# wuyakuma/HIPRT-Path-Tracer

Hardware: AMD Instinct MI355X
Metric: Mray/s + Msample/s, Bistro 1920×1080, 1/2/4/8 MI355X; RMSE vs ref @256spp (higher is better)
Workload: dtype f32

## Files before the change

### hiprt-path-tracer_amd/csrc/mpt_kernels.hip

```cpp
#include <hip/hip_runtime.h>

#include <cfloat>
#include <cstring>
#include <initializer_list>
#include <type_traits>
#include <utility>

#include "dev_bsdf.h"
#include "mpt_internal.h"

namespace mpt {

constexpr int TB = TRAV_BLOCK;
constexpr int MAX_BOUNDARY_SKIPS = 16;
#ifndef MPT_TRACE_REFILL
#define MPT_TRACE_REFILL 32
#endif
#ifndef MPT_TRACE_BUDGET
#define MPT_TRACE_BUDGET 16
#endif
constexpr int TRACE_REFILL = MPT_TRACE_REFILL;
constexpr int TRACE_BUDGET = MPT_TRACE_BUDGET;
#ifndef MPT_TRACE_CHUNK
#define MPT_TRACE_CHUNK 256
#endif
constexpr int TRACE_CHUNK = MPT_TRACE_CHUNK;
static_assert(TRACE_CHUNK >= 64, "a refill of up to 64 lanes must fit in one new chunk");
#ifndef MPT_TRI_POSTPONE
#define MPT_TRI_POSTPONE 3
#endif
constexpr int TRI_POSTPONE = MPT_TRI_POSTPONE;
constexpr uint32_t TRI_GROUP = 0x80000000u;
constexpr int LDS_STACK = TRAV_LDS_STACK;
constexpr int SPILL_DEPTH = TRAV_SPILL_DEPTH;

DEV int lane_id() { return __lane_id(); }
DEV size_t nq_index(const DevPaths& P, int id) { return (size_t)(id & 3) * (size_t)P.nq_stride + (size_t)(id >> 2); }
DEV size_t rq_phys(const DevPaths& P, int id) {
    const int s = id / RS_RPP_HOST;
    return (size_t)(id - s * RS_RPP_HOST) * (size_t)P.n + (size_t)s;
}
DEV size_t rq_rec_at(const DevPaths& P, int s, int k) { return (size_t)k * (size_t)P.n + (size_t)s; }
DEV int wave_append(int32_t* counter, bool pred) {
    unsigned long long m = __ballot(pred);
    unsigned long long act = __ballot(1);
    int leader = __ffsll((long long)act) - 1;
    int cnt = __popcll(m);
    int base = 0;
    if (lane_id() == leader && cnt) base = atomicAdd(counter, cnt);
    base = __shfl(base, leader);
    unsigned long long lower = m & ((1ull << lane_id()) - 1ull);
    return base + __popcll(lower);
}

struct THit { int prim; float t, u, v; };

DEV uint32_t alpha_key(uint32_t pixel_seed, int bounce, int kind, int iter) {
    return wang_hash(pixel_seed ^ wang_hash((uint32_t)(bounce * 8 + kind) * 0x85EBCA77u + (uint32_t)iter * 0xC2B2AE3Du + 1u));
}
DEV float alpha_uniform(uint32_t key, int prim) {
    uint32_t h = wang_hash(key ^ ((uint32_t)prim * 0x9E3779B1u));
    h = wang_hash(h + 0x7F4A7C15u);
    return (float)(h >> 8) * (1.0f / 16777216.0f);
}
DEV bool alpha_rejects(const DevScene& S, int prim, float u, float v, uint32_t key);

#ifndef MPT_TRAV_PK
#define MPT_TRAV_PK 1
#endif
DEV uint32_t qbyte(uint32_t w0, uint32_t w1, int s) { return ((s < 4 ? w0 : w1) >> ((s & 3) * 8)) & 0xffu; }

template <bool ANY, bool STATS, bool TIE = false>
struct Trav {
    v3 o, d;
    float ix, iy, iz;
    int xr;
    float best;
    int bprim;
    float bu, bv;
    uint32_t bcls;
    uint32_t gbase, gimask, gk;
    int sp;
    int last_hit;
    uint32_t akey;
    bool alpha_on;
    int tie;

    DEV void init(v3 o_, v3 d_, int lh, float tmax, bool al, uint32_t key) {
        o = o_;
        d = d_;
        ix = 1.0f / (fabsf(d.x) > 1e-30f ? d.x : copysignf(1e-30f, d.x));
        iy = 1.0f / (fabsf(d.y) > 1e-30f ? d.y : copysignf(1e-30f, d.y));
        iz = 1.0f / (fabsf(d.z) > 1e-30f ? d.z : copysignf(1e-30f, d.z));
        int oct = (d.x > 0.0f ? 1 : 0) | (d.y > 0.0f ? 2 : 0) | (d.z > 0.0f ? 4 : 0);
        xr = oct ^ 7;
        best = ANY ? tmax : INFINITY;
        bprim = -1;
        bu = 0.0f;
        bv = 0.0f;
        bcls = 0u;
        gbase = 0;
        gimask = 1u;
        gk = 1u << (0 ^ xr);
        sp = 0;
        last_hit = lh;
        akey = key;
        alpha_on = al;
    }

    DEV void push(uint2* lds, uint32_t* spill, uint2 e) {
        if (sp < LDS_STACK) lds[sp * TB + threadIdx.x] = e;
        else { spill[2 * (sp - LDS_STACK)] = e.x; spill[2 * (sp - LDS_STACK) + 1] = e.y; }
        ++sp;
    }

    DEV bool run(const DevScene& S, const Node8* bvh_nodes, const TriRec* bvh_tris, uint2* lds, uint32_t* spill, int budget,
                 uint32_t& n_nodes, uint32_t& n_tris, uint32_t* n_slots = nullptr) {
        const float4* nodes = reinterpret_cast<const float4*>(bvh_nodes);
        const float4* tris = reinterpret_cast<const float4*>(bvh_tris);
        const int tid = threadIdx.x;
        uint32_t tbase = 0u, tmask = 0u;
        while (true) {
            if (gk == 0) {
                if (sp == 0) return true;
                if (budget <= 0) return false;
                --sp;
                uint2 e;
                if (sp < LDS_STACK) e = lds[sp * TB + tid];
                else { e.x = spill[2 * (sp - LDS_STACK)]; e.y = spill[2 * (sp - LDS_STACK) + 1]; }
                if (e.y & TRI_GROUP) { tbase = e.x; tmask = e.y & ~TRI_GROUP; }
                else { gbase = e.x; gimask = e.y & 0xffu; gk = e.y >> 8; }
            } else if (budget <= 0) {
                return false;
            }
            if (gk != 0) {
                --budget;
                int k = __builtin_ctz(gk);
                gk &= gk - 1u;
                int s = k ^ xr;
                uint32_t ni = gbase + (uint32_t)__builtin_popcount(gimask & ((1u << s) - 1u));
                if (gk) push(lds, spill, make_uint2(gbase, gimask | (gk << 8)));
                if (STATS) {
                    n_nodes++;
                    if (n_slots && lane_id() == __ffsll((long long)__ballot(1)) - 1) n_slots[0] += 64;
                }
                const float4 n0 = nodes[5 * (size_t)ni + 0];
                const float4 n1 = nodes[5 * (size_t)ni + 1];
                const float4 n2 = nodes[5 * (size_t)ni + 2];
                const float4 n3 = nodes[5 * (size_t)ni + 3];
                const float4 n4 = nodes[5 * (size_t)ni + 4];
                uint32_t eb = __float_as_uint(n0.w);
                float sx = __uint_as_float((eb & 0xffu) << 23), sy = __uint_as_float(((eb >> 8) & 0xffu) << 23),
                      sz = __uint_as_float(((eb >> 16) & 0xffu) << 23);
                uint32_t imask = eb >> 24;
                float ax = (n0.x - o.x) * ix, ay = (n0.y - o.y) * iy, az = (n0.z - o.z) * iz;
                float cx = sx * ix, cy = sy * iy, cz = sz * iz;
                uint32_t lox0 = __float_as_uint(n2.x), lox1 = __float_as_uint(n2.y);
                uint32_t loy0 = __float_as_uint(n2.z), loy1 = __float_as_uint(n2.w);
                uint32_t loz0 = __float_as_uint(n3.x), loz1 = __float_as_uint(n3.y);
                uint32_t hix0 = __float_as_uint(n3.z), hix1 = __float_as_uint(n3.w);
                uint32_t hiy0 = __float_as_uint(n4.x), hiy1 = __float_as_uint(n4.y);
                uint32_t hiz0 = __float_as_uint(n4.z), hiz1 = __float_as_uint(n4.w);
                uint32_t nx0 = ix >= 0.0f ? lox0 : hix0, nx1 = ix >= 0.0f ? lox1 : hix1;
                uint32_t fx0 = ix >= 0.0f ? hix0 : lox0, fx1 = ix >= 0.0f ? hix1 : lox1;
                uint32_t ny0 = iy >= 0.0f ? loy0 : hiy0, ny1 = iy >= 0.0f ? loy1 : hiy1;
                uint32_t fy0 = iy >= 0.0f ? hiy0 : loy0, fy1 = iy >= 0.0f ? hiy1 : loy1;
                uint32_t nz0 = iz >= 0.0f ? loz0 : hiz0, nz1 = iz >= 0.0f ? loz1 : hiz1;
                uint32_t fz0 = iz >= 0.0f ? hiz0 : loz0, fz1 = iz >= 0.0f ? hiz1 : loz1;
                uint32_t meta0 = __float_as_uint(n1.z), meta1 = __float_as_uint(n1.w);
                uint32_t hit_internal = 0u;
                uint32_t hit_tris = 0u;
#if MPT_TRAV_PK
                typedef float pf2 __attribute__((ext_vector_type(2)));
#pragma unroll
                for (int c2 = 0; c2 < 8; c2 += 2) {
                    float tn2[2], tf2[2];
#pragma unroll
                    for (int j = 0; j < 2; j++) {
                        const int c = c2 + j;
                        const pf2 qx = {(float)qbyte(nx0, nx1, c), (float)qbyte(fx0, fx1, c)};
                        const pf2 qy = {(float)qbyte(ny0, ny1, c), (float)qbyte(fy0, fy1, c)};
                        const pf2 qz = {(float)qbyte(nz0, nz1, c), (float)qbyte(fz0, fz1, c)};
                        const pf2 px = __builtin_elementwise_fma(qx, (pf2){cx, cx}, (pf2){ax, ax});
                        const pf2 py = __builtin_elementwise_fma(qy, (pf2){cy, cy}, (pf2){ay, ay});
                        const pf2 pz = __builtin_elementwise_fma(qz, (pf2){cz, cz}, (pf2){az, az});
                        tn2[j] = fmaxf(fmaxf(px.x, py.x), fmaxf(pz.x, 0.0f));
                        tf2[j] = fminf(fminf(px.y, py.y), fminf(pz.y, best));
                    }
                    const pf2 tfw = (pf2){tf2[0], tf2[1]} * (pf2){1.0000009f, 1.0000009f};
#pragma unroll
                    for (int j = 0; j < 2; j++) {
                        const int c = c2 + j;
                        bool h = tn2[j] <= tfw[j];
                        bool internal = (imask >> c) & 1u;
                        if (h && internal) hit_internal |= 1u << (c ^ xr);
                        const uint32_t mw = c < 4 ? meta0 : meta1, msh = 8u * (c & 3);
                        uint32_t lm;
                        asm("v_bfm_b32 %0, %1, %2" : "=v"(lm) : "v"((mw >> (msh + 5u)) & 7u), "v"(mw >> msh));
                        if (h) hit_tris |= lm;
                    }
                }
#else
#pragma unroll
                for (int c = 0; c < 8; c++) {
                    float tnx = fmaf((float)qbyte(nx0, nx1, c), cx, ax), tfx = fmaf((float)qbyte(fx0, fx1, c), cx, ax);
                    float tny = fmaf((float)qbyte(ny0, ny1, c), cy, ay), tfy = fmaf((float)qbyte(fy0, fy1, c), cy, ay);
                    float tnz = fmaf((float)qbyte(nz0, nz1, c), cz, az), tfz = fmaf((float)qbyte(fz0, fz1, c), cz, az);
                    float tn = fmaxf(fmaxf(tnx, tny), fmaxf(tnz, 0.0f));
                    float tf = fminf(fminf(tfx, tfy), fminf(tfz, best)) * 1.0000009f;
                    bool h = tn <= tf;
                    uint32_t meta = qbyte(meta0, meta1, c);
                    bool internal = (imask >> c) & 1u;
                    if (h && internal) hit_internal |= 1u << (c ^ xr);
                    if (h && !internal) hit_tris |= ((1u << (meta >> 5)) - 1u) << (meta & 31u);
                }
#endif
                if (hit_tris) {
                    tbase = __float_as_uint(n1.y);
                    tmask = hit_tris;
                }
                gbase = __float_as_uint(n1.x);
                gimask = imask;
                gk = hit_internal;
            }
            const int n_act = __popcll(__ballot(1));
            while (tmask) {
                if (__popcll(__ballot(1)) * TRI_POSTPONE < n_act) {
                    push(lds, spill, make_uint2(tbase, tmask | TRI_GROUP));
                    tmask = 0u;
                    break;
                }
                const uint32_t ti = tbase + (uint32_t)__builtin_ctz(tmask);
                tmask &= tmask - 1u;
                if (STATS) {
                    n_tris++;
                    if (n_slots && lane_id() == __ffsll((long long)__ballot(1)) - 1) n_slots[1] += 64;
                }
                const float4 t0 = tris[3 * (size_t)ti + 0];
                const float4 t1 = tris[3 * (size_t)ti + 1];
                const float4 t2 = tris[3 * (size_t)ti + 2];
                int prim = (int)__float_as_uint(t0.w);
                v3 e1 = mk3(t1.x, t1.y, t1.z), e2 = mk3(t2.x, t2.y, t2.z);
                v3 h = cross(d, e2);
                float a = dot(e1, h);
                if (a > -0.0000001f && a < 0.0000001f) continue;
                float f = 1.0f / a;
                v3 sv = o - mk3(t0.x, t0.y, t0.z);
                float u = f * dot(sv, h);
                if (u < 0.0f || u > 1.0f) continue;
                v3 q = cross(sv, e1);
                float v = f * dot(d, q);
                if (v < 0.0f || u + v > 1.0f) continue;
                float t = f * dot(e2, q);
                if (!(t > 0.0000001f)) continue;
                if (prim == last_hit) continue;
                const bool nearer = ANY ? (t < best || (TIE && t == best && prim < tie))
                                        : (t < best || (t == best && prim < bprim));
                if (alpha_on && __float_as_uint(t1.w) != 0u && nearer && alpha_rejects(S, prim, u, v, akey))
                    continue;
                if (ANY) {
                    if (nearer) {
                        bprim = prim; best = t; bu = u; bv = v;
                        gk = 0u; sp = 0;
                        return true;
                    }
                } else if (t < best || (t == best && prim < bprim)) {
                    best = t; bprim = prim; bu = u; bv = v; bcls = __float_as_uint(t2.w);
                }
            }
        }
    }
};

template <bool ANY, bool STATS>
DEV bool traverse(const DevScene& S, v3 o, v3 d, int last_hit, float tmax, THit& out, uint2* lds, uint32_t* spill,
                  uint32_t& n_nodes, uint32_t& n_tris, bool alpha_on = false, uint32_t akey = 0u) {
    Trav<ANY, STATS> tr;
    tr.init(o, d, last_hit, tmax, alpha_on, akey);
    tr.run(S, S.nodes, S.tris, lds, spill, 0x7fffffff, n_nodes, n_tris);
    out.prim = tr.bprim;
    out.t = tr.best;
    out.u = tr.bu;
    out.v = tr.bv;
    return tr.bprim >= 0;
}

enum TraceMode { TM_PATH = 0, TM_NEE_ANY = 1, TM_NEE_CLOSEST = 2, TM_RAW_CLOSEST = 3, TM_RAW_ANY = 4, TM_NEE_LIGHT = 5,
                 TM_NEE_LIGHT_OCC = 6, TM_LIST_ANY = 7, TM_LIST_CLOSEST = 8 };
constexpr int trace_stage(int mode) {
    return mode == TM_LIST_ANY ? TM_RAW_ANY : mode == TM_LIST_CLOSEST ? TM_RAW_CLOSEST : mode >= TM_NEE_LIGHT ? TM_NEE_CLOSEST : mode;
}

struct TraceArgs {
    DevScene S;
    DevPaths P;
    const int32_t* queue;
    const int32_t* count_ptr;
    int count_const;
    int32_t* fetch;
    const float4* raw_o;
    const float4* raw_d;
    float4* raw_hit;
    uint8_t* raw_occ;
    const uint32_t* raw_key;
    const MptFrame* F;
    int bounce;
    int alpha;
    int static_grid;
    int ext;
};
DEV uint32_t slot_pixel(const MptFrame& F, int slot, int& x, int& y);
DEV uint32_t pixel_seed(const MptFrame& F, uint32_t pix);
DEV uint32_t camera_seed(const MptFrame& F, uint32_t pix);
DEV uint32_t path_seed(const MptFrame* Fp, const DevPaths& P, int slot, bool camera);

template <int MODE, bool STATS>
__global__ __launch_bounds__(TB) __attribute__((amdgpu_waves_per_eu(
    MODE == TM_PATH ? MPT_TRACE_WAVES_PATH : (MODE == TM_LIST_ANY || MODE == TM_LIST_CLOSEST) ? MPT_TRACE_WAVES_LIST : MPT_TRACE_WAVES)))
    void k_trace(TraceArgs A) {
    __shared__ uint2 lds[LDS_STACK * TB];
    const DevScene& S = A.S;
    const DevPaths& P = A.P;
    const int count = (MODE == TM_RAW_CLOSEST || MODE == TM_RAW_ANY) ? A.count_const : *A.count_ptr;
    if (MODE == TM_NEE_LIGHT && A.static_grid && (int)(blockIdx.x * TB) >= count) return;
    uint32_t* spill = P.stack_spill + (MODE == TM_NEE_LIGHT && A.static_grid ? 0 : ((size_t)blockIdx.x * TB + threadIdx.x) * (2 * SPILL_DEPTH));
    uint32_t n_nodes = 0, n_tris = 0, n_rays = 0;
    uint32_t n_slots[2] = {0u, 0u};
    constexpr bool ANY = (MODE == TM_NEE_ANY || MODE == TM_RAW_ANY || MODE == TM_NEE_LIGHT_OCC || MODE == TM_LIST_ANY);
    constexpr bool TIE = MODE == TM_NEE_LIGHT_OCC;
    const Node8* bvh_nodes = MODE == TM_NEE_LIGHT ? S.nodes_light : S.nodes;
    const TriRec* bvh_tris = MODE == TM_NEE_LIGHT ? S.tris_light : S.tris;
    Trav<ANY, STATS, TIE> tr;
    const int n_waves = (int)gridDim.x * (TB / 64);
    const int wave_id = (int)blockIdx.x * (TB / 64) + (int)(threadIdx.x >> 6);
    int sc = (count + n_waves - 1) / max(1, n_waves);
    sc = min(TRACE_CHUNK, max(64, (sc + 63) & ~63));
    const int n_static = (int)min((long long)count, (long long)sc * n_waves);
    bool alive = false;
    bool exhausted = false;
    int ray = 0;
    int skips = 0;
    uint32_t pseed = 0u;
    bool was_inside = false;
    float qmax = 0.0f;
    int chunk_next = min(wave_id * sc, n_static);
    int chunk_end = min(chunk_next + sc, n_static);
    bool counter_done = n_static >= count;
    while (true) {
        const unsigned long long idle = __ballot(!alive);
        if (!exhausted && __popcll(idle) >= (unsigned)TRACE_REFILL) {
            const int need = __popcll(idle);
            int base = 0;
            if (MODE == TM_NEE_LIGHT && A.static_grid) {
                base = (int)(blockIdx.x * TB + (threadIdx.x & ~63u));
                exhausted = true;
            }
            int take0 = need, base1 = 0;
            if (!(MODE == TM_NEE_LIGHT && A.static_grid)) {
                base = chunk_next;
                take0 = min(need, chunk_end - chunk_next);
                chunk_next += take0;
                if (take0 < need && !counter_done) {
                    int b = 0;
                    if (lane_id() == 0) b = n_static + atomicAdd(A.fetch, TRACE_CHUNK);
                    b = __shfl(b, 0);
                    counter_done = b + TRACE_CHUNK >= count;
                    chunk_end = min(b + TRACE_CHUNK, count);
                    base1 = b;
                    chunk_next = min(b + (need - take0), chunk_end);
                } else {
                    base1 = count;
                }
                exhausted = counter_done && chunk_next >= chunk_end;
            }
            if (!alive) {
                const int r = __popcll(idle & ((1ull << lane_id()) - 1ull));
                const int i = r < take0 ? base + r : base1 + (r - take0);
                if (i < count) {
                    alive = true;
                    n_rays++;
                    float4 ro, rd;
                    if (MODE == TM_PATH) {
                        ray = A.queue ? A.queue[i] : i;
                        ro = ld_s(&P.ray_o[ray]);
                        rd = ld_s(&P.ray_d[ray]);
                        skips = 0;
                        was_inside = false;
                        if (A.alpha)
                            pseed = A.bounce == 0 ? P.seeds[ray].x : P.seeds[ray].y;
                        tr.init(mk3(ro.x, ro.y, ro.z), mk3(rd.x, rd.y, rd.z), (int)__float_as_uint(ro.w), INFINITY,
                                A.alpha != 0, A.alpha ? alpha_key(pseed, A.bounce, 0, 0) : 0u);
                    } else if (MODE == TM_NEE_ANY || MODE == TM_NEE_CLOSEST || MODE == TM_NEE_LIGHT || MODE == TM_NEE_LIGHT_OCC) {
                        if (A.ext) ray = MODE == TM_NEE_LIGHT_OCC ? P.xl_light[i] : MODE == TM_NEE_ANY ? P.xl_any[i] : P.xl_cl[i];
                        else ray = MODE == TM_NEE_LIGHT_OCC ? P.nq_light[i]
                                                            : P.nq_tgt[MODE == TM_NEE_ANY ? (size_t)i : (size_t)P.n * 3 + i];
                        ro = A.ext ? P.xq_o[ray] : ld_s(&P.nq_o[nq_index(P, ray)]);
                        rd = A.ext ? P.xq_d[ray] : ld_s(&P.nq_d[nq_index(P, ray)]);
                        qmax = rd.w;
                        const bool al = A.alpha != 0;
                        uint32_t akey = 0u;
                        if (al) akey = A.ext ? alpha_key(P.seeds[ray / P.x_per].y, A.bounce, MODE == TM_NEE_ANY ? 1 : 4, 0)
                                             : alpha_key(P.seeds[ray >> 2].y, A.bounce, (ray & 3) + 1, 0);
                        float tmax = ANY ? rd.w : INFINITY;
                        if (TIE) {
                            const float4 h = A.ext ? P.xq_hit[ray] : P.nhit[ray >> 2];
                            tmax = h.x;
                            tr.tie = (int)__float_as_uint(h.w);
                        }
                        tr.init(mk3(ro.x, ro.y, ro.z), mk3(rd.x, rd.y, rd.z), (int)__float_as_uint(ro.w), tmax, al, akey);
                        if (MODE == TM_NEE_LIGHT && S.n_light_tris == 0) tr.gk = 0u;
                    } else if (MODE == TM_LIST_ANY || MODE == TM_LIST_CLOSEST) {
                        ray = (int)rq_phys(P, A.queue[i]);
                        ro = A.raw_o[ray];
                        rd = A.raw_d[ray];
                        tr.init(mk3(ro.x, ro.y, ro.z), mk3(rd.x, rd.y, rd.z), (int)__float_as_uint(ro.w), ANY ? rd.w : INFINITY,
                                A.alpha != 0, A.alpha ? A.raw_key[ray] : 0u);
                    } else {
                        ray = i;
                        ro = A.raw_o[i];
                        rd = A.raw_d[i];
                        tr.init(mk3(ro.x, ro.y, ro.z), mk3(rd.x, rd.y, rd.z), (int)__float_as_uint(ro.w), ANY ? rd.w : INFINITY, false, 0u);
                    }
                }
            }
        }
        if (__ballot(alive) == 0) {
            if (exhausted) break;
            continue;
        }
        if (!alive) continue;
        if (!tr.run(S, bvh_nodes, bvh_tris, lds, spill, TRACE_BUDGET, n_nodes, n_tris, STATS ? n_slots : nullptr)) continue;
        const bool found = tr.bprim >= 0;
        if (MODE == TM_PATH) {
            VState vs = vs_load_s(P.vsA, P.vsB, ray);
            bool again = false;
            if (found) {
                was_inside = vs.pos > 0;
                if (was_inside) vs.dist += tr.best;
                int mi = S.mat_idx[tr.bprim];
                bool skip = vs_push(vs, mi, S.mat_prio[mi]);
                if (skip && ++skips < MAX_BOUNDARY_SKIPS) {
                    vs.dist += tr.best;
                    again = true;
                }
            }
            vs_store_s(P.vsA, P.vsB, ray, vs);
            if (again) {
                n_rays++;
                tr.init(tr.o + tr.best * tr.d, tr.d, tr.last_hit, INFINITY, A.alpha != 0,
                        A.alpha ? alpha_key(pseed, A.bounce, 0, skips) : 0u);
                continue;
            }
            st_s(&P.ray_o[ray], make_float4(tr.o.x, tr.o.y, tr.o.z, __uint_as_float((uint32_t)tr.last_hit)));
            st_s(&P.hit[ray], make_float4(tr.best, tr.bu, tr.bv, __uint_as_float((uint32_t)(found ? tr.bprim : -1))));
            st_s(&P.hit_inside[ray], (uint8_t)(was_inside ? 1 : 0));
            st_s(&P.hit_cls[ray], found ? (uint8_t)tr.bcls : (uint8_t)0xffu);
        } else if (MODE == TM_NEE_ANY) {
            if (A.ext) P.xq_occ[ray] = found ? 1 : 0;
            else st_s(&P.occ[nq_index(P, ray)], (uint8_t)(found ? 1 : 0));
        } else if (MODE == TM_NEE_CLOSEST || MODE == TM_NEE_LIGHT) {
            bool ok = found && tr.best < qmax;
            (A.ext ? P.xq_hit[ray] : P.nhit[ray >> 2]) =
                make_float4(tr.best, tr.bu, tr.bv, __uint_as_float((uint32_t)(ok ? tr.bprim : -1)));
            if (MODE == TM_NEE_LIGHT && ok) {
                if (A.ext) P.xl_light[atomicAdd(&P.counters[CTR_XLIGHT], 1)] = ray;
                else P.nq_light[atomicAdd(&P.counters[CTR_LIGHT], 1)] = ray;
            }
        } else if (MODE == TM_NEE_LIGHT_OCC) {
            if (found) (A.ext ? P.xq_hit[ray] : P.nhit[ray >> 2]).w = __uint_as_float(0xffffffffu);
        } else if (MODE == TM_RAW_ANY || MODE == TM_LIST_ANY) {
            A.raw_occ[ray] = found ? 1 : 0;
        } else {
            A.raw_hit[ray] = make_float4(tr.best, tr.bu, tr.bv, __uint_as_float((uint32_t)(found ? tr.bprim : -1)));
        }
        alive = false;
    }
    if (STATS) {
        for (int off = 32; off > 0; off >>= 1) {
            n_nodes += __shfl_xor(n_nodes, off);
            n_tris += __shfl_xor(n_tris, off);
            n_rays += __shfl_xor(n_rays, off);
            n_slots[0] += __shfl_xor(n_slots[0], off);
            n_slots[1] += __shfl_xor(n_slots[1], off);
        }
        if (lane_id() == 0) {
            unsigned long long* st = (unsigned long long*)&P.stats[trace_stage(MODE) * STATS_STRIDE];
            atomicAdd(st + 0, (unsigned long long)n_rays);
            atomicAdd(st + 1, (unsigned long long)n_nodes);
            atomicAdd(st + 2, (unsigned long long)n_tris);
            atomicAdd(st + 4, (unsigned long long)n_slots[0]);
            atomicAdd(st + 5, (unsigned long long)n_slots[1]);
        }
    }
}

DEV v3 ld3(const float* p, int i) { return mk3(p[3 * (size_t)i], p[3 * (size_t)i + 1], p[3 * (size_t)i + 2]); }
DEV v2 ld2(const float* p, int i) { return mk2(p[2 * (size_t)i], p[2 * (size_t)i + 1]); }
DEV int3 tri_idx(const DevScene& S, int p) { return make_int3(S.idx[3 * (size_t)p], S.idx[3 * (size_t)p + 1], S.idx[3 * (size_t)p + 2]); }
DEV v3 uv_interp3(const float* data, int3 t, v2 uv) { return ld3(data, t.y) * uv.x + ld3(data, t.z) * uv.y + ld3(data, t.x) * (1.0f - uv.x - uv.y); }
DEV v2 uv_interp2(const float* data, int3 t, v2 uv) { return ld2(data, t.y) * uv.x + ld2(data, t.z) * uv.y + ld2(data, t.x) * (1.0f - uv.x - uv.y); }
DEV v3 tri_normal(const DevScene& S, int p) {
    const float4* tr = reinterpret_cast<const float4*>(S.tris);
    (void)tr;
    int3 t = tri_idx(S, p);
    v3 A = ld3(S.pos, t.x), B = ld3(S.pos, t.y), C = ld3(S.pos, t.z);
    return normalize(cross(B - A, C - A));
}
DEV void tex_rgba(const DevScene& S, int ti, bool srgb, v2 uv, float out[4]) {
    int w = S.tex_dims[2 * ti], h = S.tex_dims[2 * ti + 1];
    float u = wrap01(uv.x), v = 1.0f - wrap01(uv.y);
    int x = (int)(u * (float)(w - 1)), y = (int)(v * (float)(h - 1));
    const uint8_t* p = S.tex + S.tex_off[ti] + (size_t)(x + y * w) * 4;
    uchar4 c = *reinterpret_cast<const uchar4*>(p);
    if (srgb) {
        out[0] = S.srgb[c.x]; out[1] = S.srgb[c.y]; out[2] = S.srgb[c.z]; out[3] = S.srgb[c.w];
        return;
    }
    out[0] = (float)c.x / 255.0f; out[1] = (float)c.y / 255.0f; out[2] = (float)c.z / 255.0f; out[3] = (float)c.w / 255.0f;
}
DEV bool has_tex(int ti) { return ti != MPT_NO_TEXTURE && ti != MPT_CONSTANT_EMISSIVE_TEXTURE; }
DEV v2 attr_tc(const DevScene& S, int prim, v2 uv) {
    const float4* r = S.tri_attr + 5 * (size_t)prim;
    const float4 c = r[2], d = r[3];
    return mk2(c.w, d.x) * uv.x + mk2(d.y, d.z) * uv.y + mk2(c.y, c.z) * (1.0f - uv.x - uv.y);
}
DEV bool alpha_rejects(const DevScene& S, int prim, float u, float v, uint32_t key) {
    const Mat& m = S.mats[S.mat_idx[prim]];
    float a = 1.0f;
    if (S.n_tex > 0 && has_tex(m.base_color_texture_index)) {
        v2 tc = attr_tc(S, prim, mk2(u, v));
        float r[4];
        tex_rgba(S, m.base_color_texture_index, true, tc, r);
        a = r[3];
    }
    float comp = m.alpha_opacity * a;
    return !(alpha_uniform(key, prim) < comp);
}
DEV void prop_f(const DevScene& S, float& v, v2 uv, int ti) { if (has_tex(ti)) { float r[4]; tex_rgba(S, ti, false, uv, r); v = r[0]; } }
DEV void prop_c(const DevScene& S, MptColor& v, v2 uv, int ti) { if (has_tex(ti)) { float r[4]; tex_rgba(S, ti, false, uv, r); v.r = r[0]; v.g = r[1]; v.b = r[2]; } }

DEV Col emission_of(const Mat& m) { return C3(m.emission) * m.emission_strength; }
DEV bool is_emissive(const Mat& m) {
    float k = m.emission_strength;
    return !is_zero(m.emission.r * k) || !is_zero(m.emission.g * k) || !is_zero(m.emission.b * k) || m.emissive_texture_used;
}

DEV Mat intersection_material(const DevScene& S, int mi, v2 uv, bool white_furnace) {
    Mat m = S.mats[mi];
    MptColor e;
    e.r = m.emission.r * m.emission_strength / m.emission_strength;
    e.g = m.emission.g * m.emission_strength / m.emission_strength;
    e.b = m.emission.b * m.emission_strength / m.emission_strength;
    if (S.n_tex > 0) prop_c(S, e, uv, m.emission_texture_index);
    m.emission = e;
    if (white_furnace) { m.base_color.r = 1.0f; m.base_color.g = 1.0f; m.base_color.b = 1.0f; }
    else if (S.n_tex > 0 && has_tex(m.base_color_texture_index)) {
        float r[4];
        tex_rgba(S, m.base_color_texture_index, true, uv, r);
        m.base_color.r = r[0]; m.base_color.g = r[1]; m.base_color.b = r[2];
    }
    if (S.n_tex > 0) {
        if (m.roughness_metallic_texture_index != MPT_NO_TEXTURE) {
            float r[4];
            tex_rgba(S, m.roughness_metallic_texture_index, false, uv, r);
            m.roughness = r[1];
            m.metallic = r[2];
        } else {
            prop_f(S, m.metallic, uv, m.metallic_texture_index);
            prop_f(S, m.roughness, uv, m.roughness_texture_index);
        }
        prop_f(S, m.oren_nayar_sigma, uv, m.oren_sigma_texture_index);
        prop_f(S, m.specular, uv, m.specular_texture_index);
        prop_f(S, m.specular_tint, uv, m.specular_tint_texture_index);
        prop_c(S, m.specular_color, uv, m.specular_color_texture_index);
        prop_f(S, m.anisotropy, uv, m.anisotropic_texture_index);
        prop_f(S, m.anisotropy_rotation, uv, m.anisotropic_rotation_texture_index);
        prop_f(S, m.coat, uv, m.coat_texture_index);
        prop_f(S, m.coat_roughness, uv, m.coat_roughness_texture_index);
        prop_f(S, m.coat_ior, uv, m.coat_ior_texture_index);
        prop_f(S, m.sheen, uv, m.sheen_texture_index);
        prop_f(S, m.sheen_roughness, uv, m.sheen_roughness_texture_index);
        prop_c(S, m.sheen_color, uv, m.sheen_color_texture_index);
        prop_f(S, m.specular_transmission, uv, m.specular_transmission_texture_index);
    }
    float coat = m.coat;
    m.emissive_texture_used = m.emission_texture_index > 0;
    float tbr = sqrtf(sqrtf(minr(1.0f, pow4(m.roughness) + 2.0f * pow4(m.coat_roughness))));
    m.roughness = lerpr(m.roughness, lerpr(m.roughness, tbr, coat), m.coat_roughening);
    float tsr = sqrtf(sqrtf(minr(1.0f, pow4(m.second_roughness) + 2.0f * pow4(m.coat_roughness))));
    m.second_roughness = lerpr(m.second_roughness, lerpr(m.second_roughness, tsr, coat), m.coat_roughening);
    return m;
}

DEV v3 normal_mapped(const DevScene& S, const Mat& m, v3 n, int p, v2 tc) {
    int3 t = tri_idx(S, p);
    v2 d1 = ld2(S.uv, t.y) - ld2(S.uv, t.x), d2 = ld2(S.uv, t.z) - ld2(S.uv, t.x);
    v3 e1 = ld3(S.pos, t.y) - ld3(S.pos, t.x), e2 = ld3(S.pos, t.z) - ld3(S.pos, t.x);
    float di = 1.0f / (d1.x * d2.y - d1.y * d2.x);
    v3 T = (e1 * d2.y - e2 * d1.y) * di;
    v3 B = (e2 * d1.x - e1 * d2.x) * di;
    float r[4];
    tex_rgba(S, m.normal_map_texture_index, false, tc, r);
    v3 ts = normalize(mk3(r[0] - 0.5f, r[1] - 0.5f, r[2] - 0.5f));
    return to_world(normalize(T), normalize(B), n, ts);
}
DEV v3 shading_normal_of(const DevScene& S, v3 gn, int p, v2 uv, v2 tc) {
    int3 t = tri_idx(S, p);
    const Mat& m = S.mats[S.mat_idx[p]];
    v3 n = S.has_n[t.x] ? normalize(uv_interp3(S.nrm, t, uv)) : gn;
    if (S.n_tex > 0 && m.normal_map_texture_index != MPT_NO_TEXTURE) n = normal_mapped(S, m, n, p, tc);
    return n;
}

struct HitAttr { v2 tc; v3 gn, sn; int mi; };
DEV HitAttr hit_attributes(const DevScene& S, int prim, v2 uv) {
    const float4* r = S.tri_attr + 5 * (size_t)prim;
    const float4 a = r[0], b = r[1], c = r[2], d = r[3], e = r[4];
    const v3 n0 = mk3(a.x, a.y, a.z), n1 = mk3(a.w, b.x, b.y), n2 = mk3(b.z, b.w, c.x);
    const v2 t0 = mk2(c.y, c.z), t1 = mk2(c.w, d.x), t2 = mk2(d.y, d.z);
    HitAttr h;
    h.tc = t1 * uv.x + t2 * uv.y + t0 * (1.0f - uv.x - uv.y);
    h.gn = normalize(mk3(e.x, e.y, e.z));
    h.mi = __float_as_int(e.w);
    v3 n = __float_as_uint(d.w) ? normalize(n1 * uv.x + n2 * uv.y + n0 * (1.0f - uv.x - uv.y)) : h.gn;
    if (S.n_tex > 0) {
        const Mat& m = S.mats[h.mi];
        if (m.normal_map_texture_index != MPT_NO_TEXTURE) n = normal_mapped(S, m, n, prim, h.tc);
    }
    h.sn = n;
    return h;
}
#ifndef MPT_TU_PART
__global__ void k_tri_attr(DevScene S, float4* out) {
    const int p = blockIdx.x * blockDim.x + threadIdx.x;
    if (p >= S.n_tris) return;
    const int3 t = tri_idx(S, p);
    const v3 n0 = ld3(S.nrm, t.x), n1 = ld3(S.nrm, t.y), n2 = ld3(S.nrm, t.z);
    const v2 t0 = ld2(S.uv, t.x), t1 = ld2(S.uv, t.y), t2 = ld2(S.uv, t.z);
    const v3 g = tri_normal(S, p);
    float4* r = out + 5 * (size_t)p;
    r[0] = make_float4(n0.x, n0.y, n0.z, n1.x);
    r[1] = make_float4(n1.y, n1.z, n2.x, n2.y);
    r[2] = make_float4(n2.z, t0.x, t0.y, t1.x);
    r[3] = make_float4(t1.y, t2.x, t2.y, __uint_as_float(S.has_n[t.x] ? 1u : 0u));
    r[4] = make_float4(g.x, g.y, g.z, __int_as_float(S.mat_idx[p]));
}

#endif
DEV uint32_t slot_pixel(const MptFrame& F, int slot, int& x, int& y) {
    int r = slot / F.res_x;
    x = slot - r * F.res_x;
    int bh = F.band_height;
    y = ((r / bh) * F.band_count + F.band_index) * bh + (r % bh);
    return (uint32_t)x + (uint32_t)y * (uint32_t)F.res_x;
}
DEV uint32_t pixel_seed(const MptFrame& F, uint32_t pix, uint32_t random_seed) {
    const MptRenderSettings& rs = F.render_settings;
    return rs.freeze_random ? wang_hash(pix + 1u) : wang_hash((pix + 1u) * (uint32_t)(rs.sample_number + 1) * random_seed);
}
DEV uint32_t pixel_seed(const MptFrame& F, uint32_t pix) { return pixel_seed(F, pix, F.random_seed); }
DEV uint32_t camera_seed(const MptFrame& F, uint32_t pix) {
    return pixel_seed(F, pix, F.camera_random_seed ? F.camera_random_seed : F.random_seed);
}
DEV int bounce_lss(const MptFrame& F, int bounce) {
    const int lss = F.options.direct_light_sampling;
    if (lss != MPT_LSS_RESTIR_DI || bounce == 0) return lss;
    switch (F.options.restir_di_later_bounces_sampling_strategy) {
    case MPT_RESTIR_DI_LATER_BOUNCES_UNIFORM_ONE_LIGHT: return MPT_LSS_UNIFORM_ONE_LIGHT;
    case MPT_RESTIR_DI_LATER_BOUNCES_BSDF: return MPT_LSS_BSDF;
    case MPT_RESTIR_DI_LATER_BOUNCES_MIS_LIGHT_BSDF: return MPT_LSS_MIS_LIGHT_BSDF;
    default: return MPT_LSS_RIS_BSDF_AND_LIGHT;
    }
}
DEV void batch_split(const DevPaths& P, int slot, int& pix, int& sub) {
    if (P.batch == 1) { pix = slot; sub = 0; return; }
    const int g = P.group;
    const int q = slot / g;
    const int grp = q / P.batch;
    sub = q - grp * P.batch;
    pix = grp * g + (slot - q * g);
}
DEV int batch_slot(const DevPaths& P, int pix, int sub) {
    const int g = P.group;
    const int grp = pix / g;
    return (grp * P.batch + sub) * g + (pix - grp * g);
}
DEV uint32_t path_seed(const MptFrame* Fp, const DevPaths& P, int slot, bool camera) {
    int pix, sub;
    batch_split(P, slot, pix, sub);
    const MptFrame& F = Fp[sub];
    int x, y;
    const uint32_t gpix = slot_pixel(F, pix, x, y);
    return camera ? camera_seed(F, gpix) : pixel_seed(F, gpix);
}

DEV bool has_adaptive_buffers(const MptRenderSettings& rs) {
    return (rs.stop_pixel_noise_threshold > 0.0f || rs.enable_adaptive_sampling) && rs.accumulate;
}
DEV bool low_res(const MptRenderSettings& rs) {
    return rs.wants_render_low_resolution && rs.allow_render_low_resolution && rs.accumulate;
}
DEV bool low_res_region(const MptFrame& F, int x, int y) {
    const MptRenderSettings& rs = F.render_settings;
    const int s = rs.render_low_resolution_scaling;
    return x < (F.res_x + s - 1) / s && y < (F.res_y + s - 1) / s;
}
DEV float pixel_confidence(Col c, float sq, int count, float& avg) {
    float l = lum(c);
    avg = l / (float)(count + 1);
    float var = (sq - l * avg) / (float)(count + 1);
    return 1.96f * sqrtf(var) / sqrtf((float)(count + 1));
}
DEV bool adaptive_gate(const MptRenderSettings& rs, Col c, float sq, int cnt, int& conv, bool& converged) {
    if (!has_adaptive_buffers(rs)) return true;
    if (rs.enable_adaptive_sampling) {
        if (conv != -1) return false;
        if (cnt > rs.adaptive_sampling_min_samples) {
            float avg;
            float ci = pixel_confidence(c, sq, cnt, avg);
            if (!(ci > rs.adaptive_sampling_noise_threshold * avg)) {
                if (conv == -1) conv = cnt;
                return false;
            }
        }
        return true;
    } else if (rs.stop_pixel_noise_threshold > 0.0f && rs.enable_pixel_stop_noise_threshold) {
        float avg;
        float ci = pixel_confidence(c, sq, cnt, avg);
        converged = (ci <= rs.stop_pixel_noise_threshold * avg) && (rs.sample_number > 1);
        if (converged && conv == -1) conv = cnt;
        else if (!converged) conv = -1;
    }
    return true;
}
// ... 2323 lines not shown
```

Baseline: 3534.

## Traverse any-hit rays far-first, shrink their budget, add optional stack cull

Any-hit (shadow/occlusion) rays now visit child nodes in far-to-near octant order instead of near-first, and use a smaller per-iteration traversal budget before the wave regroups. A compile-time-disabled option stores a quantized near distance for child groups on the traversal stack, so closest-hit traversal can skip popped groups farther than the current best hit. This is meant to reduce wasted node visits and lane divergence for occlusion rays, at the cost of more frequent refill and scheduling passes.

```diff
diff --git a/hiprt-path-tracer_amd/csrc/mpt_kernels.hip b/hiprt-path-tracer_amd/csrc/mpt_kernels.hip
--- a/hiprt-path-tracer_amd/csrc/mpt_kernels.hip
+++ b/hiprt-path-tracer_amd/csrc/mpt_kernels.hip
@@ -21,6 +21,12 @@
 #endif
 constexpr int TRACE_REFILL = MPT_TRACE_REFILL;
 constexpr int TRACE_BUDGET = MPT_TRACE_BUDGET;
+#ifndef MPT_TRACE_REFILL_ANY
+#define MPT_TRACE_REFILL_ANY MPT_TRACE_REFILL
+#endif
+#ifndef MPT_TRACE_BUDGET_ANY
+#define MPT_TRACE_BUDGET_ANY 8
+#endif
 #ifndef MPT_TRACE_CHUNK
 #define MPT_TRACE_CHUNK 256
 #endif
@@ -68,10 +74,18 @@
 #ifndef MPT_TRAV_PK
 #define MPT_TRAV_PK 1
 #endif
+#ifndef MPT_TRAV_FAR_ANY
+#define MPT_TRAV_FAR_ANY 1
+#endif
+#ifndef MPT_TRAV_POPCULL
+#define MPT_TRAV_POPCULL 0
+#endif
+constexpr uint32_t GROUP_BOUND = 0x7fff0000u;
 DEV uint32_t qbyte(uint32_t w0, uint32_t w1, int s) { return ((s < 4 ? w0 : w1) >> ((s & 3) * 8)) & 0xffu; }
 
-template <bool ANY, bool STATS, bool TIE = false>
+template <bool ANY, bool STATS, bool TIE = false, bool POPCULL = true, bool FAR = true>
 struct Trav {
+    static constexpr bool CULL = !ANY && POPCULL && MPT_TRAV_POPCULL != 0;
     v3 o, d;
     float ix, iy, iz;
     int xr;
@@ -80,6 +94,7 @@
     float bu, bv;
     uint32_t bcls;
     uint32_t gbase, gimask, gk;
+    uint32_t gb;
     int sp;
     int last_hit;
     uint32_t akey;
@@ -93,7 +108,7 @@
         iy = 1.0f / (fabsf(d.y) > 1e-30f ? d.y : copysignf(1e-30f, d.y));
         iz = 1.0f / (fabsf(d.z) > 1e-30f ? d.z : copysignf(1e-30f, d.z));
         int oct = (d.x > 0.0f ? 1 : 0) | (d.y > 0.0f ? 2 : 0) | (d.z > 0.0f ? 4 : 0);
-        xr = oct ^ 7;
+        xr = (ANY && FAR && MPT_TRAV_FAR_ANY) ? oct : oct ^ 7;
         best = ANY ? tmax : INFINITY;
         bprim = -1;
         bu = 0.0f;
@@ -102,6 +117,7 @@
         gbase = 0;
         gimask = 1u;
         gk = 1u << (0 ^ xr);
+        gb = 0u;
         sp = 0;
         last_hit = lh;
         akey = key;
@@ -121,15 +137,27 @@
         const int tid = threadIdx.x;
         uint32_t tbase = 0u, tmask = 0u;
         while (true) {
+            if (CULL && gk != 0) {
+                const float bw = best * 1.0000009f;
+                if (__uint_as_float(gb & GROUP_BOUND) > bw) { gk &= gk - 1u; gb = (gb << 16) | (gb & 0xffffu); }
+                if (__uint_as_float(gb & GROUP_BOUND) > bw) gk = 0u;
+            }
             if (gk == 0) {
                 if (sp == 0) return true;
                 if (budget <= 0) return false;
-                --sp;
-                uint2 e;
-                if (sp < LDS_STACK) e = lds[sp * TB + tid];
-                else { e.x = spill[2 * (sp - LDS_STACK)]; e.y = spill[2 * (sp - LDS_STACK) + 1]; }
-                if (e.y & TRI_GROUP) { tbase = e.x; tmask = e.y & ~TRI_GROUP; }
-                else { gbase = e.x; gimask = e.y & 0xffu; gk = e.y >> 8; }
+                while (true) {
+                    --sp;
+                    uint2 e;
+                    if (sp < LDS_STACK) e = lds[sp * TB + tid];
+                    else { e.x = spill[2 * (sp - LDS_STACK)]; e.y = spill[2 * (sp - LDS_STACK) + 1]; }
+                    if (e.y & TRI_GROUP) { tbase = e.x; tmask = e.y & ~TRI_GROUP; break; }
+                    gbase = e.x; gimask = e.y & 0xffu; gk = (e.y >> 8) & 0xffu;
+                    if (!CULL) break;
+                    gb = (e.y & GROUP_BOUND) | ((e.y >> 16) & 0x7fffu);
+                    if (!(__uint_as_float(e.y & GROUP_BOUND) > best * 1.0000009f)) break;
+                    gk = 0u;
+                    if (sp == 0) return true;
+                }
             } else if (budget <= 0) {
                 return false;
             }
@@ -139,7 +167,7 @@
                 gk &= gk - 1u;
                 int s = k ^ xr;
                 uint32_t ni = gbase + (uint32_t)__builtin_popcount(gimask & ((1u << s) - 1u));
-                if (gk) push(lds, spill, make_uint2(gbase, gimask | (gk << 8)));
+                if (gk) push(lds, spill, make_uint2(gbase, gimask | (gk << 8) | (CULL ? (gb << 16) & GROUP_BOUND : 0u)));
                 if (STATS) {
                     n_nodes++;
                     if (n_slots && lane_id() == __ffsll((long long)__ballot(1)) - 1) n_slots[0] += 64;
@@ -170,6 +198,8 @@
                 uint32_t meta0 = __float_as_uint(n1.z), meta1 = __float_as_uint(n1.w);
                 uint32_t hit_internal = 0u;
                 uint32_t hit_tris = 0u;
+                constexpr uint32_t NO_CHILD = 0x7f800000u;
+                uint32_t m1 = NO_CHILD, m2 = NO_CHILD;
 #if MPT_TRAV_PK
                 typedef float pf2 __attribute__((ext_vector_type(2)));
 #pragma unroll
@@ -194,6 +224,11 @@
                         bool h = tn2[j] <= tfw[j];
                         bool internal = (imask >> c) & 1u;
                         if (h && internal) hit_internal |= 1u << (c ^ xr);
+                        if (CULL) {
+                            const uint32_t key = (h && internal) ? (__float_as_uint(tn2[j]) & ~7u) | (uint32_t)(c ^ xr) : NO_CHILD;
+                            m2 = min(m2, max(m1, key));
+                            m1 = min(m1, key);
+                        }
                         const uint32_t mw = c < 4 ? meta0 : meta1, msh = 8u * (c & 3);
                         uint32_t lm;
                         asm("v_bfm_b32 %0, %1, %2" : "=v"(lm) : "v"((mw >> (msh + 5u)) & 7u), "v"(mw >> msh));
@@ -212,6 +247,11 @@
                     uint32_t meta = qbyte(meta0, meta1, c);
                     bool internal = (imask >> c) & 1u;
                     if (h && internal) hit_internal |= 1u << (c ^ xr);
+                    if (CULL) {
+                        const uint32_t key = (h && internal) ? (__float_as_uint(tn) & ~7u) | (uint32_t)(c ^ xr) : NO_CHILD;
+                        m2 = min(m2, max(m1, key));
+                        m1 = min(m1, key);
+                    }
                     if (h && !internal) hit_tris |= ((1u << (meta >> 5)) - 1u) << (meta & 31u);
                 }
 #endif
@@ -222,6 +262,10 @@
                 gbase = __float_as_uint(n1.x);
                 gimask = imask;
                 gk = hit_internal;
+                if (CULL) {
+                    const uint32_t rest = (int)(m1 & 7u) == __builtin_ctz(hit_internal | 0x100u) ? m2 : m1;
+                    gb = (m1 & GROUP_BOUND) | ((rest >> 16) & 0x7fffu);
+                }
             }
             const int n_act = __popcll(__ballot(1));
             while (tmask) {
@@ -275,7 +319,7 @@
 template <bool ANY, bool STATS>
 DEV bool traverse(const DevScene& S, v3 o, v3 d, int last_hit, float tmax, THit& out, uint2* lds, uint32_t* spill,
                   uint32_t& n_nodes, uint32_t& n_tris, bool alpha_on = false, uint32_t akey = 0u) {
-    Trav<ANY, STATS> tr;
+    Trav<ANY, STATS, false, false, false> tr;
     tr.init(o, d, last_hit, tmax, alpha_on, akey);
     tr.run(S, S.nodes, S.tris, lds, spill, 0x7fffffff, n_nodes, n_tris);
     out.prim = tr.bprim;
@@ -330,7 +374,8 @@
     constexpr bool TIE = MODE == TM_NEE_LIGHT_OCC;
     const Node8* bvh_nodes = MODE == TM_NEE_LIGHT ? S.nodes_light : S.nodes;
     const TriRec* bvh_tris = MODE == TM_NEE_LIGHT ? S.tris_light : S.tris;
-    Trav<ANY, STATS, TIE> tr;
+    Trav<ANY, STATS, TIE, MODE != TM_NEE_LIGHT && MODE != TM_NEE_CLOSEST, MODE != TM_LIST_ANY> tr;
+    constexpr bool SHORT = ANY && MODE != TM_LIST_ANY;
     const int n_waves = (int)gridDim.x * (TB / 64);
     const int wave_id = (int)blockIdx.x * (TB / 64) + (int)(threadIdx.x >> 6);
     int sc = (count + n_waves - 1) / max(1, n_waves);
@@ -348,7 +393,7 @@
     bool counter_done = n_static >= count;
     while (true) {
         const unsigned long long idle = __ballot(!alive);
-        if (!exhausted && __popcll(idle) >= (unsigned)TRACE_REFILL) {
+        if (!exhausted && __popcll(idle) >= (unsigned)(SHORT ? MPT_TRACE_REFILL_ANY : TRACE_REFILL)) {
             const int need = __popcll(idle);
             int base = 0;
             if (MODE == TM_NEE_LIGHT && A.static_grid) {
@@ -429,7 +474,7 @@
             continue;
         }
         if (!alive) continue;
-        if (!tr.run(S, bvh_nodes, bvh_tris, lds, spill, TRACE_BUDGET, n_nodes, n_tris, STATS ? n_slots : nullptr)) continue;
+        if (!tr.run(S, bvh_nodes, bvh_tris, lds, spill, SHORT ? MPT_TRACE_BUDGET_ANY : TRACE_BUDGET, n_nodes, n_tris, STATS ? n_slots : nullptr)) continue;
         const bool found = tr.bprim >= 0;
         if (MODE == TM_PATH) {
             VState vs = vs_load_s(P.vsA, P.vsB, ray);
```

New measurement: 3578, median of 6. +1.2%, better.
